# huahbo/IBAMR

Measured on AMD Instinct MI355X. Metric: IB_4 3D spread+interp marker-ops/sec (fp64) + % HBM roofline, 1/2/4/8 GPU, higher is better.
Workload: dtype f64; 1 GPU; cfg4: 1024^3 periodic staggered grid, 1e8 uniform markers (seed 1234), IB_4, z-slabs; kernel=IB_4, markers=100000000, parallelism=z-slab x1, marker_order=cell, layout=packed, spread_mode=one rank, move=False, renumber=False, spread_into=zeroed f (LDataManager::spread, LDataManager.cpp:596), overlap=False

## Files before the change

### ibamr_amd/csrc/le_abi.cpp

```cpp
#include <hip/hip_runtime.h>

#include <algorithm>
#include <climits>
#include <cmath>
#include <cstdlib>
#include <cstdarg>
#include <cstdio>
#include <cstring>
#include <string>
#include <unordered_map>
#include <vector>

#include "../../include/ibtk_le.h"
#include "le_internal.h"

using namespace ibtk_le;

static thread_local std::string g_last_error;

static int fail(int code, const char* fmt, ...) {
    char buf[512];
    va_list ap;
    va_start(ap, fmt);
    vsnprintf(buf, sizeof(buf), fmt, ap);
// ... 129 lines not shown
    int kernel = -1;
    int ndim = 0;
    BinGeom bg{};
    ColGeom cg{};
    int S = 0, nseg = 0;
    ibtk_le_patch_geom geom{};
    DevBuf sorted_key, sorted_l, sorted_s, sorted_X, sorted_a, plane_start, indices, xshift;
    DevBuf sorted_X2, xcur;
    bool xcur_set = false;
    DevBuf lvl_nbr;
    std::vector<int2> lvl_nbr_host;
    DevBuf cand_cnt, cand_off, cand_idx;
    DevBuf last, qdst;
    DevBuf items, nsub, isub, nitems;
    DevBuf cs_cnt, cs_off, cs_pos;
    int cs_state = 0;
    const int* cs_skip = nullptr;
    DevBuf cs_off_z;
    bool cs_split = false;
    long long nclz = 0;
    DevBuf zbits, zst;
    int rb_epoch = 0;
    int item_bound = 0;
    int npatch = 0;
    std::vector<ibtk_le_patch_geom> geoms;
    std::vector<PatchDesc> pdh;
    std::vector<PatchDesc> pdh_dev;
    std::vector<int> off_dev;
    DevBuf pd, entry_off;
    int nbuckets_total = 0, njobs = 0;
// ... 103 lines not shown
extern "C" int ibtk_le_ctx_tune(ibtk_le_ctx ctx, const char* key, int value) {
    if (!ctx || !key) return fail(IBTK_LE_ERR_ARG, "null argument");
    SweepTune& t = ctx->tune;
    const std::string k = key;
    if (k == "seg_items") t.seg_items = value;
    else if (k == "split_target") t.split_target = value;
    else if (k == "heavy") t.heavy = value;
    else if (k == "min_piece") t.min_piece = value;
    else if (k == "heavy_target") t.heavy_target = value;
    else if (k == "heavy_min_piece") t.heavy_min_piece = value;
    else if (k == "heavy_first") t.heavy_first = value;
    else if (k == "strip") t.strip = value;
    else if (k == "xcd_block") t.xcd_block = value;
    else if (k == "interp3") t.interp3 = value;
    else if (k == "side_gather") t.side_gather = value;
    else return fail(IBTK_LE_ERR_ARG, "unknown tuning key %s", key);
    return IBTK_LE_OK;
}

extern "C" int ibtk_le_ctx_enable_timing(ibtk_le_ctx ctx, int enable) {
    if (!ctx) return fail(IBTK_LE_ERR_ARG, "null ctx");
    ctx->timing = enable != 0;
    return IBTK_LE_OK;
}

extern "C" double ibtk_le_ctx_last_kernel_ms(ibtk_le_ctx ctx) {
    if (!ctx || !ctx->ev_valid) return -1.0;
    hipEventSynchronize(ctx->ev1);
    float ms = -1.f;
    if (hipEventElapsedTime(&ms, ctx->ev0, ctx->ev1) != hipSuccess) return -1.0;
// ... 209 lines not shown
    *out = m;
    return IBTK_LE_OK;
}

extern "C" int ibtk_le_markers_destroy(ibtk_le_markers m) {
    if (!m) return IBTK_LE_OK;
    hipSetDevice(m->ctx->device);
    hipStreamSynchronize(m->ctx->stream);
    for (DevBuf* b : {&m->sorted_X2, &m->xcur, &m->lvl_nbr})
        b->release();
    for (DevBuf* b : {&m->sorted_key, &m->sorted_l, &m->sorted_s, &m->sorted_X, &m->sorted_a, &m->plane_start, &m->indices,
                      &m->xshift, &m->cand_cnt, &m->cand_off, &m->cand_idx, &m->last, &m->qdst, &m->items,
                      &m->nsub, &m->isub, &m->nitems, &m->pd, &m->entry_off, &m->qin, &m->owner, &m->int_off,
                      &m->rb_cin, &m->rb_cout, &m->rb_d, &m->rb_dpre, &m->rb_mstart, &m->rb_ps2, &m->rb_mbits,
                      &m->rb_wcnt, &m->rb_wpre, &m->rb_mlist, &m->rb_scr, &m->rb_big, &m->rb_nbig, &m->cs_cnt,
                      &m->cs_off, &m->cs_pos, &m->cs_off_z, &m->zbits, &m->zst, &m->sel_gs})
        b->release();
    delete m;
    return IBTK_LE_OK;
}

extern "C" int ibtk_le_markers_count(ibtk_le_markers m) { return m ? m->n : -1; }

extern "C" int ibtk_le_markers_order(ibtk_le_markers m, const int** order_dev) {
    if (!m || !order_dev) return fail(IBTK_LE_ERR_ARG, "markers_order: null argument");
    *order_dev = m->sorted_l.as<int>();
    return IBTK_LE_OK;
}

#ifndef IBTK_LE_STRIP
#define IBTK_LE_STRIP 1
// ... 525 lines not shown
    if ((rc = m->cand_cnt.ensure(sizeof(int) * (size_t)(items + 1)))) return rc;
    if ((rc = m->cand_off.ensure(sizeof(int) * (size_t)(items + 1)))) return rc;
    if ((rc = m->cand_idx.ensure(sizeof(int) * (size_t)m->n * (m->ndim == 3 ? 8 : 4)))) return rc;
    HIP_TRY(hipMemsetAsync(m->cand_cnt.p, 0, sizeof(int) * (size_t)(items + 1), s));
    HIP_TRY(launch_cand(m->ndim, m->kernel, p, false, m->cand_cnt.as<int>(), nullptr, s));
    size_t tb = 0;
    HIP_TRY(launch_scan(nullptr, tb, m->cand_cnt.as<int>(), m->cand_off.as<int>(), items + 1, s));
    if ((rc = ctx->temp.ensure(tb))) return rc;
    tb = ctx->temp.cap;
    HIP_TRY(launch_scan(ctx->temp.p, tb, m->cand_cnt.as<int>(), m->cand_off.as<int>(), items + 1, s));
    HIP_TRY(launch_cand(m->ndim, m->kernel, p, true, m->cand_off.as<int>(), m->cand_idx.as<int>(), s));
    m->cand_valid = true;
    return IBTK_LE_OK;
}

static bool side_gather(ibtk_le_ctx ctx, ibtk_le_markers m) {
    const int t = ctx->tune.side_gather;
    return t > 0 || (t == 0 && m->n >= (1 << 25));
}
static int gather_fork(ibtk_le_ctx ctx, const Params& p) {
    if (!ctx->side) {
        if (!ctx->ev_fork) HIP_TRY(hipEventCreateWithFlags(&ctx->ev_fork, hipEventDisableTiming));
        if (!ctx->ev_join) HIP_TRY(hipEventCreateWithFlags(&ctx->ev_join, hipEventDisableTiming));
        hipStream_t st = nullptr;
        HIP_TRY(hipStreamCreateWithFlags(&st, hipStreamNonBlocking));
        ctx->side = st;
    }
    HIP_TRY(hipEventRecord(ctx->ev_fork, ctx->stream));
    HIP_TRY(hipStreamWaitEvent(ctx->side, ctx->ev_fork, 0));
    HIP_TRY(launch_gather_F(p, ctx->side));
    HIP_TRY(hipEventRecord(ctx->ev_join, ctx->side));
    return IBTK_LE_OK;
}
// ... 195 lines not shown

extern "C" int ibtk_le_user_interp(ibtk_le_ctx ctx, int centering, int axis, const ibtk_le_patch_geom* geom,
                                   const double* const* q_dev, int q_depth, double* Q_dev, int Q_depth,
                                   const double* X_dev, const int* indices_dev, const double* Xshift_dev, int n) {
    return user_call(ctx, false, centering, axis, geom, const_cast<double* const*>(q_dev), q_depth, Q_dev, Q_depth, X_dev,
                     indices_dev, Xshift_dev, n);
}
extern "C" int ibtk_le_user_spread(ibtk_le_ctx ctx, int centering, int axis, const ibtk_le_patch_geom* geom,
                                   double* const* q_dev, int q_depth, const double* Q_dev, int Q_depth,
                                   const double* X_dev, const int* indices_dev, const double* Xshift_dev, int n) {
    return user_call(ctx, true, centering, axis, geom, q_dev, q_depth, const_cast<double*>(Q_dev), Q_depth, X_dev,
                     indices_dev, Xshift_dev, n);
}

static bool cand_split(int k) { return k == K_IB_4 || k == K_BSPLINE_4 || k == K_IB_6 || k == K_IB_4_W8; }
static bool cand_stream_built(ibtk_le_markers m) {
    return m->cs_state == 1 && m->cs_pos.p && (m->cs_split || !cand_split(m->kernel));
}
static int cand_stream(ibtk_le_ctx ctx, ibtk_le_markers m, Params& p) {
    const long long ncl = (long long)m->nbuckets_total / NBAND;
    const long long nclz = m->npatch ? m->nclz : (long long)m->cg.ncol * (m->cg.nz + 1);
    const int k = m->kernel;
    const bool split = cand_split(k);
    const long long cap = std::min(std::max(4LL * m->n, 1LL), (1LL << 31) - 1);
    if (ncl + 1 >= (1LL << 31) || nclz + 1 >= (1LL << 31))
        return fail(IBTK_LE_ERR_RANGE, "candidate stream too long");
    p.cs_off = m->cs_off.as<int>();
    p.cs_pos = m->cs_pos.as<int>();
    p.cs_total = (int)cap;
    p.cs_off_z = m->cs_split ? m->cs_off_z.as<int>() : nullptr;
    p.cs_rint = k == K_IB_4 ? 1 : 0;
    if (cand_stream_built(m)) return IBTK_LE_OK;
    int rc;
    const size_t tot_at = (sizeof(int) * (size_t)(ncl + 1) + 7) / 8 * 8;
    if ((rc = m->cs_cnt.ensure(tot_at + sizeof(unsigned long long)))) return rc;
    if ((rc = m->cs_off.ensure(sizeof(int) * (size_t)(ncl + 1)))) return rc;
    if ((rc = m->cs_pos.ensure(sizeof(int) * (size_t)cap))) return rc;
    if (split && (rc = m->cs_off_z.ensure(sizeof(int) * (size_t)(nclz + 1)))) return rc;
    p.cs_off = m->cs_off.as<int>();
    p.cs_pos = m->cs_pos.as<int>();
    p.cs_off_z = split ? m->cs_off_z.as<int>() : nullptr;
    HIP_TRY(hipMemsetAsync(m->cs_cnt.as<int>() + ncl, 0, sizeof(int), ctx->stream));
    size_t tb = 0;
    HIP_TRY(launch_scan(nullptr, tb, m->cs_cnt.as<int>(), m->cs_off.as<int>(), (int)(ncl + 1), ctx->stream));
    if ((rc = ctx->temp.ensure(tb))) return rc;
    Params q = p;
    const bool keep = m->cs_state == 2 && (!split || (m->cs_split && m->zst.p));
    q.items_skip = keep ? m->cs_skip : nullptr;
    q.cs_zflip = m->zst.p ? m->zst.as<int>() + 1 : nullptr;
    q.cs_epoch = m->rb_epoch;
    HIP_TRY(launch_cand_stream(q, (int)ncl, m->cs_cnt.as<int>(), m->cs_off.as<int>(), m->cs_pos.as<int>(), ctx->temp.p,
                               ctx->temp.cap,
                               reinterpret_cast<unsigned long long*>(m->cs_cnt.as<char>() + tot_at), ctx->stream));
    m->cs_state = 1;
    m->cs_split = split;
    return IBTK_LE_OK;
}

static int spread_impl(ibtk_le_ctx ctx, ibtk_le_markers m, int kernel, int centering, int axis,
                       const ibtk_le_patch_geom* geom, double* const* q_dev, int q_depth, const double* Q_dev,
                       int Q_depth, const double* ds_dev, const double* X_dev, bool zero_ghosts, bool zero_first) {
    Params p;
    if (int rc = prepare(ctx, m, kernel, geom, X_dev, p)) return rc;
    p.zero_ghosts = zero_ghosts ? 1 : 0;
    p.zero_first = zero_first ? 1 : 0;
    const int nc = ncomponents(geom, centering, q_depth, Q_depth);
    if (nc < 0) return -nc;
    if (m->n == 0) return IBTK_LE_OK;
    if (!Q_dev || !q_dev) return fail(IBTK_LE_ERR_ARG, "null Q or q");
    if (set_device(ctx)) return IBTK_LE_ERR_DEVICE;
    p.Qin = Q_dev;
    p.ds = ds_dev;
    p.Q_depth = Q_depth;
    p.nsorted = m->n;
    {
        if (int rc = ctx->fbuf.ensure(sizeof(double) * (size_t)m->n * (size_t)std::min(nc, MAXC))) return rc;
        p.sorted_F = ctx->fbuf.as<double>();
    }
    if (geom->ndim == 2) {
        if (int rc = build_candidates(ctx, m, p)) return rc;
        p.cand_off = m->cand_off.as<int>();
        p.cand_idx = m->cand_idx.as<int>();
    }
    ctx->ev_valid = false;
    for (int first = 0; first < nc; first += MAXC) {
        const int cnt = std::min(MAXC, nc - first);
        if (int rc = make_comps(geom, centering, axis, q_dev, q_depth, Q_depth, first, cnt, p)) return rc;
        const bool side = geom->ndim == 3 && side_gather(ctx, m) && !cand_stream_built(m);
        if (side)
            if (int rc = gather_fork(ctx, p)) return rc;
        if (geom->ndim == 3)
            if (int rc = cand_stream(ctx, m, p)) return rc;
        if (side)
            if (int rc = gather_join(ctx)) return rc;
        const bool t = ctx->timing && first == 0;
        const size_t nst = (size_t)m->item_bound * cnt * 8;
        if (geom->ndim == 3)
            if (int rc = stamps_begin(ctx, nst, p)) return rc;
        if (geom->ndim == 3) {
            if (int rc = adds_begin(ctx, p, first == 0)) return rc;
            HIP_TRY(launch_spread_sweep(kernel, p, ctx->stream, t ? ctx->ev0 : nullptr, t ? ctx->ev1 : nullptr,
                                        !side));
            if (int rc = adds_end(ctx, p)) return rc;
// ... 294 lines not shown
}

static int level_spread_impl(ibtk_le_ctx ctx, ibtk_le_markers m, int kernel, int centering, int axis,
                             double* const* q_dev, int q_depth, const double* Q_dev, int Q_depth, const double* X_dev,
                             bool zero_first) {
    Params p;
    std::memset(&p, 0, sizeof(p));
    int nc = 0;
    if (int rc = level_params(ctx, m, kernel, centering, axis, q_dev, q_depth, Q_depth, X_dev, false, p, nc))
        return rc;
    if (m->n == 0)
        return zero_first ? ibtk_le_level_zero(ctx, m->npatch, m->geoms.data(), centering, q_dev, q_depth) : IBTK_LE_OK;
    if (!Q_dev) return fail(IBTK_LE_ERR_ARG, "null Q");
    p.Qin = Q_dev;
    p.zero_first = zero_first ? 1 : 0;
    {
        if (int rc = ctx->fbuf.ensure(sizeof(double) * (size_t)m->n * (size_t)nc)) return rc;
        p.sorted_F = ctx->fbuf.as<double>();
    }
    const bool side = side_gather(ctx, m) && !cand_stream_built(m);
    if (side)
        if (int rc = gather_fork(ctx, p)) return rc;
    if (int rc = cand_stream(ctx, m, p)) return rc;
    if (side)
        if (int rc = gather_join(ctx)) return rc;
    const bool t = ctx->timing;
    ctx->ev_valid = false;
    const size_t nst = (size_t)m->item_bound * nc * 8;
    if (int rc = stamps_begin(ctx, nst, p)) return rc;
    if (int rc = adds_begin(ctx, p, true)) return rc;
    HIP_TRY(launch_spread_sweep(kernel, p, ctx->stream, t ? ctx->ev0 : nullptr, t ? ctx->ev1 : nullptr, !side));
    if (int rc = adds_end(ctx, p)) return rc;
    if (int rc = stamps_report(ctx, nst, p)) return rc;
    if (t) ctx->ev_valid = true;
    return IBTK_LE_OK;
// ... 1269 lines not shown
```

### ibamr_amd/csrc/le_internal.h

```cpp
#pragma once
#include <hip/hip_runtime.h>

#include <cstdint>

namespace ibtk_le {

enum : int {
    K_PIECEWISE_CONSTANT = 0,
    K_DISCONTINUOUS_LINEAR = 1,
    K_PIECEWISE_LINEAR = 2,
    K_PIECEWISE_CUBIC = 3,
    K_IB_3 = 4,
    K_IB_4 = 5,
    K_IB_4_W8 = 6,
    K_IB_6 = 7,
    K_BSPLINE_4 = 8,
    K_COUNT = 9
};

struct KernelInfo {
    int W, LO, HI;
};
constexpr KernelInfo kKernelInfo[K_COUNT] = {
    {1, 0, 1},
// ... 53 lines not shown
    int nbuckets;
};

struct SweepTune {
    int seg_items = 0;
    int split_target = 0;
    int heavy = 0;
    int strip = 0;
    int xcd_block = 0;
    int min_piece = 0;
    int heavy_target = 0;
    int heavy_min_piece = 0;
    int heavy_first = 0;
    int interp3 = 0;
    int side_gather = 0;
};
struct SweepItem {
    int col, p0, p1, patch;
};
struct PatchDesc {
    ColGeom cg;
    int bucket_base;
    int ca_base_z;
    int jbase;
    int S, nseg;
    double xlo[3];
    int ilower[3];
    CompDesc comp[MAXC];
};

// ... 21 lines not shown
    double h3;
    double K6;
    const double* X;
    const int* indices;
    const double* Xshift;
    const int* sorted_l;
    const int* sorted_s;
    const double* sorted_X;
    const double* const* sorted_X_ref;
    const unsigned* sorted_key;
    const int* plane_start;
    const int* cand_off;
    const int* cand_idx;
    const int* cs_off;
    const int* cs_pos;
    int cs_total;
    const int* cs_off_z;
    int cs_rint;
    const int* cs_zflip;
    int cs_epoch;
    const int* nentries_dev;
    const double* Qin;
    const double* sorted_F;
    const double* ds;
    int nsorted;
    double* Qout;
    const int* qdst;
    int* err;
    double* sink;
    const int* n_dev = nullptr;
// ... 99 lines not shown
    const void* trec;
    const double *X, *dX, *U;
    double* F;
    int accumulate;
};
hipError_t launch_forcegen(int ndim, const ForceGenParams& p, hipStream_t s);
hipError_t launch_gather_col(int kernel, const Params& p, int n, int* sorted_s, double* sorted_X,
                             const unsigned* sorted_key, int nbuckets, int* bucket_start, hipStream_t s);
hipError_t launch_interp_sweep(int kernel, const Params& p, int n, hipStream_t s, hipEvent_t ev0, hipEvent_t ev1);
hipError_t launch_spread_sweep(int kernel, const Params& p, hipStream_t s, hipEvent_t ev0, hipEvent_t ev1,
                               bool gather = true);
hipError_t launch_gather_F(const Params& p, hipStream_t s);
void sweep_segments(const ColGeom& cg, int& S, int& nseg, int seg_items, bool level);
hipError_t launch_item_table(int kernel, const Params& p, int target, int heavy, int* nsub, int* start, SweepItem* tab, int* ntot,
                             void* temp, size_t temp_bytes, hipStream_t s);
hipError_t launch_cand_stream(const Params& p, int ncl, int* cnt, int* off, int* pos, void* temp, size_t temp_bytes,
                              unsigned long long* total, hipStream_t s);

struct GhostDesc {
    double* u;
    int lo[3], hi[3];
    int ilo[3], ihi[3];
    int64_t s1, s2;
};
constexpr int GSET = 4;
struct GhostSet {
    GhostDesc g[GSET];
};
hipError_t launch_fill_periodic(int ndim, const GhostDesc* g, int n, const int* periodic, hipStream_t s);
hipError_t launch_fold_periodic(int ndim, const GhostDesc* g, int n, const int* periodic, hipStream_t s);
hipError_t launch_zero_ghosts(int ndim, const GhostDesc* g, int n, hipStream_t s);

// ... 133 lines not shown
```

### ibamr_amd/csrc/le_sweep.hip

```cpp
#include <hip/hip_runtime.h>

#include <climits>
#include <type_traits>
#include <cstdio>
#include <cstdlib>

#include "le_internal.h"
#include "le_stencil.h"

namespace ibtk_le {

constexpr int SW = 64;
#ifndef IBTK_LE_DIAG_SPREAD
#define IBTK_LE_DIAG_SPREAD 0
#endif

__device__ __forceinline__ double lds_ld(const double* q) {
    return *(const volatile __attribute__((address_space(3))) double*)q;
}

__device__ __forceinline__ int lane_id() { return __lane_id(); }

struct D3 {
    double v[3];
// ... 1250 lines not shown
            }
        }
        cnt[ca] = t;
    }
}
struct CaJob {
    ColGeom cg;
    int col, a, zb, zilo, o, t;
    double zxlo;
    bool items;
    const int* bs;
    int rowv[3];
    Ranges R;
    int e0;
    double z0;
};
template <bool SHZ>
__global__ __launch_bounds__(BLOCK) void k_cand_write(Params p, int ncl, const int* off, int* pos,
                                                      const unsigned long long* total) {
    if (cs_stands(p)) return;
    if (*total >= (unsigned long long)p.cs_total + 1ull) {
        if (blockIdx.x == 0 && threadIdx.x == 0) atomicOr(p.err, 16);
        return;
    }
    const int lane = threadIdx.x & (SW - 1);
    const int nw = gridDim.x * (BLOCK / SW);
    gdouble* const sX = cur_sorted_X(p);
    const double inv_dz = 1.0 / p.bg.dx[2];
    int* const offz = const_cast<int*>(p.cs_off_z);
    __shared__ int ptab_s[CS_PTAB];
    const int* const ptab = cs_patch_table(p, ptab_s);
    auto load_rows = [&](int ca, CaJob& J) {
        J.items = ca < ncl && ca_decode(p, ca, J.cg, J.col, J.a, J.bs, J.zb, J.zxlo, J.zilo, ptab);
        J.o = off[min(ca, ncl - 1)];
        if (p.pd) J.items = J.items && off[min(ca + 1, ncl)] != J.o;
        if (J.items) {
            const int cx = J.col % J.cg.ncx, cy = J.col / J.cg.ncx;
            const int col0 = (cy - 1) * J.cg.ncx + (cx - 1);
#pragma unroll
            for (int r = 0; r < 3; ++r) J.rowv[r] = J.bs[bucket(J.cg, J.a, col0 + r * J.cg.ncx, 0) + min(lane, 27)];
        }
    };
    auto load_first = [&](CaJob& J) {
        J.t = 0;
        J.e0 = 0;
        J.z0 = 0.0;
        if (!J.items) return;
        make_ranges_lanes(J.rowv, J.R);
        J.t = J.R.pre[SSh<K_IB_4>::NR];
        J.e0 = range_pos(J.R, min(lane, max(J.t - 1, 0)));
        if constexpr (SHZ) J.z0 = sX[(int64_t)3 * min(J.e0, p.nsorted - 1) + 2];
    };
    auto finish = [&](int ca, CaJob& J) {
        if (ca >= ncl) return;
        const int o = J.o;
        if (SHZ && lane == 0) {
            if (J.a == 0) offz[J.zb] = o;
            if (ca == ncl - 1) offz[J.zb + 2] = off[ca + 1];
        }
        const int t = J.t;
        if constexpr (!SHZ) {
            if (lane < t) pos[o + lane] = J.e0;
            for (int j = lane + SW; j < t; j += SW) pos[o + j] = range_pos(J.R, j);
        } else {
            const int aa = J.a + J.cg.org[2] - J.zilo;
            int nlo = 0, nup = 0;
            for (int j0 = 0; j0 < t; j0 += SW) {
                const int j = j0 + lane;
                int e = J.e0;
                double z = J.z0;
                if (j0 > 0) {
                    e = range_pos(J.R, min(j, t - 1));
                    z = sX[(int64_t)3 * e + 2];
                }
                const double xo = (z - J.zxlo) * inv_dz;
                const int n = p.cs_rint ? (int)__builtin_rint(xo) : d_nint(xo);
                const bool in = j < t;
                const bool up = in && n > aa;
                const unsigned long long bu = __ballot(up), bl = __ballot(in && !up);
                const unsigned long long below = (1ull << lane) - 1ull;
                if (in) {
                    if (up) pos[o + t - 1 - (nup + __popcll(bu & below))] = e;
                    else pos[o + nlo + __popcll(bl & below)] = e;
                }
                nlo += __popcll(bl);
                nup += __popcll(bu);
            }
            if (lane == 0) offz[J.zb + 1] = o + nlo;
        }
    };
    for (int ca = blockIdx.x * (BLOCK / SW) + (int)(threadIdx.x / SW); ca < ncl; ca += nw) {
        CaJob J;
        load_rows(ca, J);
        load_first(J);
        finish(ca, J);
    }
}
hipError_t launch_cand_stream(const Params& p, int ncl, int* cnt, int* off, int* pos, void* temp, size_t temp_bytes,
                              unsigned long long* total, hipStream_t s) {
    if (ncl <= 0) return hipSuccess;
    hipLaunchKernelGGL(k_cand_count, dim3(std::min((ncl + BLOCK - 1) / BLOCK, CS_GRID)), dim3(BLOCK), 0, s, p, ncl,
                       cnt);
    hipError_t e = hipMemsetAsync(total, 0, sizeof(unsigned long long), s);
    if (e != hipSuccess) return e;
    if (p.cs_total >= 0x7fffffff && (e = launch_sum64(cnt, ncl, total, s)) != hipSuccess) return e;
    e = launch_scan(temp, temp_bytes, cnt, off, ncl + 1, s);
    if (e != hipSuccess) return e;
    const int per = BLOCK / SW;
    const dim3 g(std::min((ncl + per - 1) / per, CS_GRID)), b(BLOCK);
    if (p.cs_off_z) hipLaunchKernelGGL(k_cand_write<true>, g, b, 0, s, p, ncl, off, pos, total);
    else hipLaunchKernelGGL(k_cand_write<false>, g, b, 0, s, p, ncl, off, pos, total);
    return hipGetLastError();
}

struct Cand {
    double X[3];
    double V;
    int s;
};

template <typename T> __device__ __forceinline__ void rot4(T* w, int r) {
    const bool b0 = r & 1, b1 = r & 2;
    const T c0 = b0 ? w[1] : w[0], c1 = b0 ? w[2] : w[1], c2 = b0 ? w[3] : w[2], c3 = b0 ? w[0] : w[3];
    w[0] = b1 ? c2 : c0;
    w[1] = b1 ? c3 : c1;
    w[2] = b1 ? c0 : c2;
// ... 218 lines not shown
    }
}
template <int K, bool CNT, bool ZC, typename Before>
__device__ __forceinline__ void spread_tiled(const Params& p, const CompDesc& cd, double* ring, const Cand& cdat,
                                             bool act, int a, int X0, int Y0, int zorg, int xlo, int xhi, int ylo,
                                             int yhi, int plo, int phi, double inv_h3, const double* inv_d, Clk& clk,
                                             unsigned long long* cnt, Before&& before) {
    TileAdds<SSh<K, ZC>::W> T;
    spread_setup<K, CNT, ZC>(p, cd, cdat, act, a, X0, Y0, zorg, xlo, xhi, ylo, yhi, plo, phi, inv_h3, inv_d, cnt,
                             before, T);
    clk.lap(2);
    spread_adds<K, ZC>(ring, T);
    clk.lap(3);
}

template <int K, bool LVL, bool CNT, bool ZC>
__global__ __launch_bounds__(SW) void k_spread_sweep(Params p) {
    using S = SSh<K, ZC>;
    constexpr int LO = S::LO, HI = S::HIE, NPL = S::NPL, FAM = S::FAM;
    __shared__ double ring[S::NSL * S::PV];
    const int it = sweep_item(p, p.ncomp);
    if (it < 0) return;
    int c;
    SweepItem si;
    item_decode(p, it, c, si);
    c += p.comp0;
    const int col = si.col;
    const int lane = lane_id();
    ColGeom cg;
    CompDesc cd;
    const int* bs;
// ... 6 lines not shown
    const int zorg = cg.org[2];
    const int xlo = max(cd.lo[0] - X0, 0), xhi = min(cd.hi[0] - X0, COLX - 1);
    const int ylo = max(cd.lo[1] - Y0, 0), yhi = min(cd.hi[1] - Y0, COLY - 1);
    const int plo = max(si.p0, cd.lo[2] - zorg), phi = min(si.p1 - 1, cd.hi[2] - zorg);
    if (xlo > xhi || ylo > yhi || plo > phi) return;
    if (p.zmode) {
        const bool inner = zorg + plo >= p.zlo && zorg + phi <= p.zhi;
        if (inner != (p.zmode == 1)) return;
    }
    const bool shz = FAM == 0 && !cd.zcell;
    static_assert(ZC || FAM != 0, "closed-form kernels: every component on the key-frame ring");
    const int nza = shz ? cg.nz + 1 : cg.nz;
    const int afirst = max(plo - HI, 0), alast = min(phi - LO, nza - 1);
    const int* const cs_offs = shz ? p.cs_off_z : p.cs_off;
    const int ca0 = (LVL ? (shz ? p.pd[si.patch].ca_base_z : p.pd[si.patch].bucket_base / NBAND) : 0) + col * nza + afirst;
    const bool any = cs_offs[ca0 + (alast - afirst + 1)] > cs_offs[ca0];
    const bool zg = p.zero_ghosts && !p.zero_first;
    int dlo[3], dhi[3];
#pragma unroll
    for (int d = 0; d < 3; ++d) {
        dlo[d] = cd.ilower[d];
        dhi[d] = cd.iupper[d];
    }
    const bool xy_inner = X0 >= dlo[0] && X0 + COLX - 1 <= dhi[0] && Y0 >= dlo[1] && Y0 + COLY - 1 <= dhi[1];
    const bool z_inner = zorg + plo >= dlo[2] && zorg + phi <= dhi[2];
    if (!any && !p.zero_first && !(zg && !(xy_inner && z_inner))) return;
    const int nlast = p.nsorted - 1;
    unsigned loff[NPL];
    unsigned gmask = 0;
#pragma unroll
    for (int k = 0; k < NPL; ++k) {
// ... 7 lines not shown
    auto zghost = [&](int z) { return zorg + z < dlo[2] || zorg + z > dhi[2]; };
    const unsigned plane_bytes = (unsigned)(8 * cd.s2);
    auto plane_ptr = [&](int z) {
        const int zc = min(max(zorg + z, cd.lo[2]), cd.hi[2]);
        return plane_rsrc(cd.u + (int64_t)(zc - cd.lo[2]) * cd.s2, plane_bytes);
    };
    if (!any) {
        for (int z = plo; z <= phi; ++z) {
            const auto pb = plane_ptr(z);
            const bool all = p.zero_first || zghost(z);
#pragma unroll
            for (int k = 0; k < NPL; ++k) buf_st(pb, (all || ((gmask >> k) & 1u)) ? loff[k] : OFF_NONE, 0.0);
        }
        return;
    }
    auto cand_at = [&](int e, Cand& d) {
        e = min(max(e, 0), nlast);
#if IBTK_LE_DIAG_SPREAD & 8
        d.X[0] = d.X[1] = d.X[2] = 0.5 + 1e-9 * e;
        d.V = 1.0;
        d.s = 0;
        return;
#endif
        const D3 xs = ld3(sorted_X + (int64_t)3 * e);
        d.X[0] = xs.v[0];
        d.X[1] = xs.v[1];
        d.X[2] = xs.v[2];
        d.V = p.sorted_F[(int64_t)c * p.nsorted + e];
        d.s = FAM == 2 ? p.sorted_s[e] : 0;
    };
    Clk clk;
    unsigned long long cnt[2] = {0ull, 0ull};
    const double inv_h3 = 1.0 / p.h3;
    const double inv_d[3] = {1.0 / p.bg.dx[0], 1.0 / p.bg.dx[1], 1.0 / p.bg.dx[2]};
    auto process = [&](int a, int r, int n, const Cand& mine, auto&& before) {
#if IBTK_LE_DIAG_SPREAD & 4
        asm volatile("" ::"v"(mine.X[0]), "v"(mine.X[1]), "v"(mine.X[2]), "v"(mine.V));
        before();
#else
        spread_tiled<K, CNT, ZC>(p, cd, ring, mine, lane < n, lane < r ? a - 1 : a, X0, Y0, zorg, xlo, xhi, ylo, yhi, plo, phi,
                             inv_h3, inv_d, clk, cnt, before);
#endif
    };
    auto nothing = [] {};
// ... 33 lines not shown
    auto wb_read = [&](int z, double* v) {
        const double* sl = ring + sslot<S>(z) * S::PV;
#pragma unroll
        for (int k = 0; k < NPL; ++k) v[k] = sl[lane + k * SW];
    };
    auto wb_store = [&](int z, bool on, const double* v) {
        const int zc = min(max(zorg + z, cd.lo[2]), cd.hi[2]);
        const bool own = on && z >= plo && z <= phi;
        const auto pb = plane_rsrc(cd.u + (int64_t)(zc - cd.lo[2]) * cd.s2, own ? plane_bytes : 0u);
#pragma unroll
        for (int k = 0; k < NPL; ++k) buf_st(pb, loff[k], v[k]);
    };

    clk.start(p.stamps != nullptr);
    const int* const cs_pos = p.cs_pos;
    const int cs_last = p.cs_total - 1;
    const int nk = alast - afirst + 1;
    auto off_load = [&](int k) { return cs_offs[ca0 + min(k, nk)]; };
    auto pos_load = [&](int j) { return cs_pos[min(max(j, 0), cs_last)]; };
    double pv[NPL] = {};
    for (int z = afirst + LO; z < afirst + HI; ++z) {
        plane_load(z, pv);
        plane_put(z, pv);
    }
    plane_load(afirst + HI, pv);
    int O0 = __builtin_amdgcn_readfirstlane(off_load(0)), O1 = __builtin_amdgcn_readfirstlane(off_load(1));
    int O2 = __builtin_amdgcn_readfirstlane(off_load(2)), O3 = __builtin_amdgcn_readfirstlane(off_load(3));
    int O4v = off_load(4);
    int R0 = 0;
    int N0 = min(O1 - O0, SW);
    int R1 = (O1 - O0 - N0) % SW;
    int N1 = R1 + min(SW - R1, O2 - O1);
    Cand nxt, nxt2;
    {
        const int e0 = pos_load(O0 + min(lane, max(N0 - 1, 0)));
        cand_at(e0, nxt);
    }
    int I1 = pos_load(O1 - R1 + min(lane, max(N1 - 1, 0)));
    clk.lap(0);
    auto anchor_step = [&](int a, const Cand& cur, Cand& nxt) __attribute__((always_inline)) {
        const int k = a - afirst;
        const int zw = a - 2 + LO;
        double wb[NPL];
        wb_read(zw, wb);
        plane_put(a + HI, pv);
        asm volatile("" ::"v"(cur.X[0]), "v"(cur.X[1]), "v"(cur.X[2]), "v"(cur.V), "v"(I1), "v"(O4v));
        const int O4 = __builtin_amdgcn_readfirstlane(O4v);
        const int cur_r = R0, cur_n = N0;
        const int tCur = O1 - O0;
        const int h = min(SW - R0, tCur);
        const int nmid = (tCur - h) / SW;
        const int r_a = R1;
        clk.lap(1);
        int R2 = 0, N2 = 0;
        if (a + 1 <= alast) {
            cand_at(I1, nxt);
            const int t1 = O2 - O1;
            R2 = (t1 - min(SW - R1, t1)) % SW;
            N2 = R2 + min(SW - R2, O3 - O2);
            I1 = pos_load(O2 - R2 + min(lane, max(N2 - 1, 0)));
            O4v = off_load(k + 5);
            plane_load(a + HI + 1, pv);
        }
        const bool wbon = a >= afirst + 2;
        if (cur_n > 0) process(a, cur_r, cur_n, cur, [&] { wb_store(zw, wbon, wb); });
        else wb_store(zw, wbon, wb);
        if (nmid > 0) {
            const int mbase = O0 + h + lane;
            Cand more, more2;
            cand_at(pos_load(mbase), more);
            int m = 0;
            if constexpr (PAIR) {
                if (nmid > 1) cand_at(pos_load(mbase + SW), more2);
                int q2 = pos_load(mbase + SW * 2), q3 = pos_load(mbase + SW * 3);
                for (; m + 1 < nmid; m += 2) {
                    const Cand n0 = more, n1 = more2;
                    if (m + 2 < nmid) cand_at(q2, more);
                    if (m + 3 < nmid) cand_at(q3, more2);
                    q2 = pos_load(mbase + SW * (m + 4));
                    q3 = pos_load(mbase + SW * (m + 5));
                    process2(a, n0, n1);
                }
            }
            int q1 = pos_load(mbase + SW * (m + 1));
            for (; m < nmid; ++m) {
                const Cand now = more;
                if (m + 1 < nmid) cand_at(q1, more);
                q1 = pos_load(mbase + SW * (m + 2));
                process(a, 0, SW, now, nothing);
            }
        }
        if (a == alast && r_a > 0) {
            Cand last;
            cand_at(pos_load(O1 - r_a + min(lane, r_a - 1)), last);
            process(a, 0, r_a, last, nothing);
        }
        R0 = R1;
        N0 = N1;
        R1 = R2;
        N1 = N2;
        O0 = O1;
        O1 = O2;
        O2 = O3;
        O3 = O4;
        clk.lap(4);
    };
    for (int a = afirst; a <= alast; ++a) {
        anchor_step(a, nxt, nxt2);
        nxt = nxt2;
// ... 248 lines not shown
    }
}

hipError_t launch_gather_F(const Params& p, hipStream_t s) {
    if (p.nsorted > 0) {
        const bool rec3 = p.ncomp == 3 && p.Q_depth == 3 && p.comp[0].qcomp == 0 && p.comp[1].qcomp == 1 &&
                          p.comp[2].qcomp == 2;
        const dim3 g((p.nsorted + BLOCK - 1) / BLOCK), b(BLOCK);
        if (rec3) hipLaunchKernelGGL(k_gather_F_col<true>, g, b, 0, s, p, p.nsorted, const_cast<double*>(p.sorted_F));
        else hipLaunchKernelGGL(k_gather_F_col<false>, g, b, 0, s, p, p.nsorted, const_cast<double*>(p.sorted_F));
    }
    return hipGetLastError();
}
template <int K>
hipError_t launch_spread_sweep_t(const Params& p, hipStream_t s, hipEvent_t ev0, hipEvent_t ev1, bool gather) {
    if (gather)
        if (hipError_t e = launch_gather_F(p, s); e != hipSuccess) return e;
    if (ev0) (void)hipEventRecord(ev0, s);
    const long items = (long)p.item_bound * p.ncomp;
    if (items > 0) {
        Params q = p;
        q.comp0 = 0;
        const dim3 g(sweep_grid(q, items)), b(SW);
        constexpr bool ZC = KT<K>::FAM == 0;
        if (q.nadd) {
            if (q.pd) hipLaunchKernelGGL((k_spread_sweep<K, true, true, ZC>), g, b, 0, s, q);
            else hipLaunchKernelGGL((k_spread_sweep<K, false, true, ZC>), g, b, 0, s, q);
        } else {
            if (q.pd) hipLaunchKernelGGL((k_spread_sweep<K, true, false, ZC>), g, b, 0, s, q);
            else hipLaunchKernelGGL((k_spread_sweep<K, false, false, ZC>), g, b, 0, s, q);
        }
    }
    if (ev1) (void)hipEventRecord(ev1, s);
    return hipGetLastError();
}

#define IBTK_LE_DISPATCH_K(KV, CALL)                                 \
    switch (KV) {                                                    \
    case K_PIECEWISE_CONSTANT: return CALL<K_PIECEWISE_CONSTANT>;    \
    case K_DISCONTINUOUS_LINEAR: return CALL<K_DISCONTINUOUS_LINEAR>; \
    case K_PIECEWISE_LINEAR: return CALL<K_PIECEWISE_LINEAR>;        \
    case K_PIECEWISE_CUBIC: return CALL<K_PIECEWISE_CUBIC>;          \
    case K_IB_3: return CALL<K_IB_3>;                                \
    case K_IB_4: return CALL<K_IB_4>;                                \
    case K_IB_4_W8: return CALL<K_IB_4_W8>;                          \
    case K_IB_6: return CALL<K_IB_6>;                                \
// ... 100 lines not shown
```

Measured before the change: 8.330 billion marker-ops/s.

## Stream marker source indices in candidate list to skip separate force gather pass

The candidate-stream builder now also records each candidate's original marker index (cs_src). The spread sweep kernel, under a new FS template flag, reads force values straight from Qin (scaled by ds) through that index, so the separate gather pass into sorted_F and its side-stream overlap are dropped. It is on by default (f_stream defaults to 0, so the test >= 0 holds). This saves one pass that writes and then rereads an n×ncomp buffer. In exchange it adds an extra int stream load per candidate and turns coalesced sorted reads into scattered reads of Qin.

```diff
diff --git a/ibamr_amd/csrc/le_abi.cpp b/ibamr_amd/csrc/le_abi.cpp
--- a/ibamr_amd/csrc/le_abi.cpp
+++ b/ibamr_amd/csrc/le_abi.cpp
@@ -167,6 +167,8 @@
     DevBuf last, qdst;
     DevBuf items, nsub, isub, nitems;
     DevBuf cs_cnt, cs_off, cs_pos;
+    DevBuf cs_src;
+    bool cs_has_src = false;
     int cs_state = 0;
     const int* cs_skip = nullptr;
     DevBuf cs_off_z;
@@ -300,6 +302,7 @@
     else if (k == "xcd_block") t.xcd_block = value;
     else if (k == "interp3") t.interp3 = value;
     else if (k == "side_gather") t.side_gather = value;
+    else if (k == "f_stream") t.f_stream = value;
     else return fail(IBTK_LE_ERR_ARG, "unknown tuning key %s", key);
     return IBTK_LE_OK;
 }
@@ -539,7 +542,7 @@
                       &m->nsub, &m->isub, &m->nitems, &m->pd, &m->entry_off, &m->qin, &m->owner, &m->int_off,
                       &m->rb_cin, &m->rb_cout, &m->rb_d, &m->rb_dpre, &m->rb_mstart, &m->rb_ps2, &m->rb_mbits,
                       &m->rb_wcnt, &m->rb_wpre, &m->rb_mlist, &m->rb_scr, &m->rb_big, &m->rb_nbig, &m->cs_cnt,
-                      &m->cs_off, &m->cs_pos, &m->cs_off_z, &m->zbits, &m->zst, &m->sel_gs})
+                      &m->cs_off, &m->cs_pos, &m->cs_src, &m->cs_off_z, &m->zbits, &m->zst, &m->sel_gs})
         b->release();
     delete m;
     return IBTK_LE_OK;
@@ -1095,9 +1098,12 @@
     return IBTK_LE_OK;
 }
 
+static bool f_stream(ibtk_le_ctx ctx, ibtk_le_markers) {
+    return ctx->tune.f_stream >= 0;
+}
 static bool side_gather(ibtk_le_ctx ctx, ibtk_le_markers m) {
     const int t = ctx->tune.side_gather;
-    return t > 0 || (t == 0 && m->n >= (1 << 25));
+    return !f_stream(ctx, m) && (t > 0 || (t == 0 && m->n >= (1 << 25)));
 }
 static int gather_fork(ibtk_le_ctx ctx, const Params& p) {
     if (!ctx->side) {
@@ -1323,46 +1329,51 @@
 }
 
 static bool cand_split(int k) { return k == K_IB_4 || k == K_BSPLINE_4 || k == K_IB_6 || k == K_IB_4_W8; }
-static bool cand_stream_built(ibtk_le_markers m) {
-    return m->cs_state == 1 && m->cs_pos.p && (m->cs_split || !cand_split(m->kernel));
+static bool cand_stream_built(ibtk_le_markers m, bool src) {
+    return m->cs_state == 1 && m->cs_pos.p && (m->cs_split || !cand_split(m->kernel)) && (!src || m->cs_has_src);
 }
 static int cand_stream(ibtk_le_ctx ctx, ibtk_le_markers m, Params& p) {
     const long long ncl = (long long)m->nbuckets_total / NBAND;
     const long long nclz = m->npatch ? m->nclz : (long long)m->cg.ncol * (m->cg.nz + 1);
     const int k = m->kernel;
     const bool split = cand_split(k);
+    const bool src = f_stream(ctx, m);
     const long long cap = std::min(std::max(4LL * m->n, 1LL), (1LL << 31) - 1);
     if (ncl + 1 >= (1LL << 31) || nclz + 1 >= (1LL << 31))
         return fail(IBTK_LE_ERR_RANGE, "candidate stream too long");
     p.cs_off = m->cs_off.as<int>();
     p.cs_pos = m->cs_pos.as<int>();
+    p.cs_src = src ? m->cs_src.as<int>() : nullptr;
     p.cs_total = (int)cap;
     p.cs_off_z = m->cs_split ? m->cs_off_z.as<int>() : nullptr;
     p.cs_rint = k == K_IB_4 ? 1 : 0;
-    if (cand_stream_built(m)) return IBTK_LE_OK;
+    if (cand_stream_built(m, src)) return IBTK_LE_OK;
     int rc;
     const size_t tot_at = (sizeof(int) * (size_t)(ncl + 1) + 7) / 8 * 8;
     if ((rc = m->cs_cnt.ensure(tot_at + sizeof(unsigned long long)))) return rc;
     if ((rc = m->cs_off.ensure(sizeof(int) * (size_t)(ncl + 1)))) return rc;
     if ((rc = m->cs_pos.ensure(sizeof(int) * (size_t)cap))) return rc;
+    if (src && (rc = m->cs_src.ensure(sizeof(int) * (size_t)cap))) return rc;
     if (split && (rc = m->cs_off_z.ensure(sizeof(int) * (size_t)(nclz + 1)))) return rc;
     p.cs_off = m->cs_off.as<int>();
     p.cs_pos = m->cs_pos.as<int>();
+    p.cs_src = src ? m->cs_src.as<int>() : nullptr;
     p.cs_off_z = split ? m->cs_off_z.as<int>() : nullptr;
     HIP_TRY(hipMemsetAsync(m->cs_cnt.as<int>() + ncl, 0, sizeof(int), ctx->stream));
     size_t tb = 0;
     HIP_TRY(launch_scan(nullptr, tb, m->cs_cnt.as<int>(), m->cs_off.as<int>(), (int)(ncl + 1), ctx->stream));
     if ((rc = ctx->temp.ensure(tb))) return rc;
     Params q = p;
-    const bool keep = m->cs_state == 2 && (!split || (m->cs_split && m->zst.p));
+    const bool keep = m->cs_state == 2 && (!split || (m->cs_split && m->zst.p)) && (!src || m->cs_has_src);
     q.items_skip = keep ? m->cs_skip : nullptr;
     q.cs_zflip = m->zst.p ? m->zst.as<int>() + 1 : nullptr;
     q.cs_epoch = m->rb_epoch;
-    HIP_TRY(launch_cand_stream(q, (int)ncl, m->cs_cnt.as<int>(), m->cs_off.as<int>(), m->cs_pos.as<int>(), ctx->temp.p,
-                               ctx->temp.cap,
+    HIP_TRY(launch_cand_stream(q, (int)ncl, m->cs_cnt.as<int>(), m->cs_off.as<int>(), m->cs_pos.as<int>(),
+                               src ? m->cs_src.as<int>() : nullptr, ctx->temp.p, ctx->temp.cap,
                                reinterpret_cast<unsigned long long*>(m->cs_cnt.as<char>() + tot_at), ctx->stream));
     m->cs_state = 1;
     m->cs_split = split;
+    m->cs_has_src = src;
     return IBTK_LE_OK;
 }
 
@@ -1382,7 +1393,8 @@
     p.ds = ds_dev;
     p.Q_depth = Q_depth;
     p.nsorted = m->n;
-    {
+    p.sorted_F = nullptr;
+    if (geom->ndim == 2 || !f_stream(ctx, m)) {
         if (int rc = ctx->fbuf.ensure(sizeof(double) * (size_t)m->n * (size_t)std::min(nc, MAXC))) return rc;
         p.sorted_F = ctx->fbuf.as<double>();
     }
@@ -1395,7 +1407,7 @@
     for (int first = 0; first < nc; first += MAXC) {
         const int cnt = std::min(MAXC, nc - first);
         if (int rc = make_comps(geom, centering, axis, q_dev, q_depth, Q_depth, first, cnt, p)) return rc;
-        const bool side = geom->ndim == 3 && side_gather(ctx, m) && !cand_stream_built(m);
+        const bool side = geom->ndim == 3 && side_gather(ctx, m) && !cand_stream_built(m, false);
         if (side)
             if (int rc = gather_fork(ctx, p)) return rc;
         if (geom->ndim == 3)
@@ -1720,11 +1732,12 @@
     if (!Q_dev) return fail(IBTK_LE_ERR_ARG, "null Q");
     p.Qin = Q_dev;
     p.zero_first = zero_first ? 1 : 0;
-    {
+    p.sorted_F = nullptr;
+    if (!f_stream(ctx, m)) {
         if (int rc = ctx->fbuf.ensure(sizeof(double) * (size_t)m->n * (size_t)nc)) return rc;
         p.sorted_F = ctx->fbuf.as<double>();
     }
-    const bool side = side_gather(ctx, m) && !cand_stream_built(m);
+    const bool side = side_gather(ctx, m) && !cand_stream_built(m, false);
     if (side)
         if (int rc = gather_fork(ctx, p)) return rc;
     if (int rc = cand_stream(ctx, m, p)) return rc;
diff --git a/ibamr_amd/csrc/le_internal.h b/ibamr_amd/csrc/le_internal.h
--- a/ibamr_amd/csrc/le_internal.h
+++ b/ibamr_amd/csrc/le_internal.h
@@ -91,6 +91,7 @@
     int heavy_first = 0;
     int interp3 = 0;
     int side_gather = 0;
+    int f_stream = 0;
 };
 struct SweepItem {
     int col, p0, p1, patch;
@@ -142,6 +143,7 @@
     const int* cand_idx;
     const int* cs_off;
     const int* cs_pos;
+    const int* cs_src = nullptr;
     int cs_total;
     const int* cs_off_z;
     int cs_rint;
@@ -271,8 +273,8 @@
 void sweep_segments(const ColGeom& cg, int& S, int& nseg, int seg_items, bool level);
 hipError_t launch_item_table(int kernel, const Params& p, int target, int heavy, int* nsub, int* start, SweepItem* tab, int* ntot,
                              void* temp, size_t temp_bytes, hipStream_t s);
-hipError_t launch_cand_stream(const Params& p, int ncl, int* cnt, int* off, int* pos, void* temp, size_t temp_bytes,
-                              unsigned long long* total, hipStream_t s);
+hipError_t launch_cand_stream(const Params& p, int ncl, int* cnt, int* off, int* pos, int* src, void* temp,
+                              size_t temp_bytes, unsigned long long* total, hipStream_t s);
 
 struct GhostDesc {
     double* u;
diff --git a/ibamr_amd/csrc/le_sweep.hip b/ibamr_amd/csrc/le_sweep.hip
--- a/ibamr_amd/csrc/le_sweep.hip
+++ b/ibamr_amd/csrc/le_sweep.hip
@@ -1288,13 +1288,17 @@
     Ranges R;
     int e0;
     double z0;
+    int s0;
 };
 template <bool SHZ>
-__global__ __launch_bounds__(BLOCK) void k_cand_write(Params p, int ncl, const int* off, int* pos,
+__global__ __launch_bounds__(BLOCK) void k_cand_write(Params p, int ncl, const int* off, int* pos, int* src,
                                                       const unsigned long long* total) {
     if (cs_stands(p)) return;
     if (*total >= (unsigned long long)p.cs_total + 1ull) {
         if (blockIdx.x == 0 && threadIdx.x == 0) atomicOr(p.err, 16);
+        if (src)
+            for (int64_t j = (int64_t)blockIdx.x * BLOCK + threadIdx.x; j < p.cs_total; j += (int64_t)gridDim.x * BLOCK)
+                src[j] = 0;
         return;
     }
     const int lane = threadIdx.x & (SW - 1);
@@ -1319,11 +1323,13 @@
         J.t = 0;
         J.e0 = 0;
         J.z0 = 0.0;
+        J.s0 = 0;
         if (!J.items) return;
         make_ranges_lanes(J.rowv, J.R);
         J.t = J.R.pre[SSh<K_IB_4>::NR];
         J.e0 = range_pos(J.R, min(lane, max(J.t - 1, 0)));
         if constexpr (SHZ) J.z0 = sX[(int64_t)3 * min(J.e0, p.nsorted - 1) + 2];
+        if (src) J.s0 = p.sorted_s[min(J.e0, p.nsorted - 1)];
     };
     auto finish = [&](int ca, CaJob& J) {
         if (ca >= ncl) return;
@@ -1336,16 +1342,21 @@
         if constexpr (!SHZ) {
             if (lane < t) pos[o + lane] = J.e0;
             for (int j = lane + SW; j < t; j += SW) pos[o + j] = range_pos(J.R, j);
+            if (src) {
+                if (lane < t) src[o + lane] = J.s0;
+                for (int j = lane + SW; j < t; j += SW) src[o + j] = p.sorted_s[min(range_pos(J.R, j), p.nsorted - 1)];
+            }
         } else {
             const int aa = J.a + J.cg.org[2] - J.zilo;
             int nlo = 0, nup = 0;
             for (int j0 = 0; j0 < t; j0 += SW) {
                 const int j = j0 + lane;
-                int e = J.e0;
+                int e = J.e0, ms = J.s0;
                 double z = J.z0;
                 if (j0 > 0) {
                     e = range_pos(J.R, min(j, t - 1));
                     z = sX[(int64_t)3 * e + 2];
+                    if (src) ms = p.sorted_s[min(e, p.nsorted - 1)];
                 }
                 const double xo = (z - J.zxlo) * inv_dz;
                 const int n = p.cs_rint ? (int)__builtin_rint(xo) : d_nint(xo);
@@ -1354,8 +1365,9 @@
                 const unsigned long long bu = __ballot(up), bl = __ballot(in && !up);
                 const unsigned long long below = (1ull << lane) - 1ull;
                 if (in) {
-                    if (up) pos[o + t - 1 - (nup + __popcll(bu & below))] = e;
-                    else pos[o + nlo + __popcll(bl & below)] = e;
+                    const int at = up ? o + t - 1 - (nup + __popcll(bu & below)) : o + nlo + __popcll(bl & below);
+                    pos[at] = e;
+                    if (src) src[at] = ms;
                 }
                 nlo += __popcll(bl);
                 nup += __popcll(bu);
@@ -1370,8 +1382,8 @@
         finish(ca, J);
     }
 }
-hipError_t launch_cand_stream(const Params& p, int ncl, int* cnt, int* off, int* pos, void* temp, size_t temp_bytes,
-                              unsigned long long* total, hipStream_t s) {
+hipError_t launch_cand_stream(const Params& p, int ncl, int* cnt, int* off, int* pos, int* src, void* temp,
+                              size_t temp_bytes, unsigned long long* total, hipStream_t s) {
     if (ncl <= 0) return hipSuccess;
     hipLaunchKernelGGL(k_cand_count, dim3(std::min((ncl + BLOCK - 1) / BLOCK, CS_GRID)), dim3(BLOCK), 0, s, p, ncl,
                        cnt);
@@ -1382,8 +1394,8 @@
     if (e != hipSuccess) return e;
     const int per = BLOCK / SW;
     const dim3 g(std::min((ncl + per - 1) / per, CS_GRID)), b(BLOCK);
-    if (p.cs_off_z) hipLaunchKernelGGL(k_cand_write<true>, g, b, 0, s, p, ncl, off, pos, total);
-    else hipLaunchKernelGGL(k_cand_write<false>, g, b, 0, s, p, ncl, off, pos, total);
+    if (p.cs_off_z) hipLaunchKernelGGL(k_cand_write<true>, g, b, 0, s, p, ncl, off, pos, src, total);
+    else hipLaunchKernelGGL(k_cand_write<false>, g, b, 0, s, p, ncl, off, pos, src, total);
     return hipGetLastError();
 }
 
@@ -1632,7 +1644,7 @@
     clk.lap(3);
 }
 
-template <int K, bool LVL, bool CNT, bool ZC>
+template <int K, bool LVL, bool CNT, bool ZC, bool FS>
 __global__ __launch_bounds__(SW) void k_spread_sweep(Params p) {
     using S = SSh<K, ZC>;
     constexpr int LO = S::LO, HI = S::HIE, NPL = S::NPL, FAM = S::FAM;
@@ -1669,7 +1681,8 @@
     const int afirst = max(plo - HI, 0), alast = min(phi - LO, nza - 1);
     const int* const cs_offs = shz ? p.cs_off_z : p.cs_off;
     const int ca0 = (LVL ? (shz ? p.pd[si.patch].ca_base_z : p.pd[si.patch].bucket_base / NBAND) : 0) + col * nza + afirst;
-    const bool any = cs_offs[ca0 + (alast - afirst + 1)] > cs_offs[ca0];
+    const int o_end = cs_offs[ca0 + (alast - afirst + 1)];
+    const bool any = o_end > cs_offs[ca0];
     const bool zg = p.zero_ghosts && !p.zero_first;
     int dlo[3], dhi[3];
 #pragma unroll
@@ -1707,7 +1720,8 @@
         }
         return;
     }
-    auto cand_at = [&](int e, Cand& d) {
+    const int* const cs_src = p.cs_src;
+    auto cand_at = [&](int e, int s, Cand& d) {
         e = min(max(e, 0), nlast);
 #if IBTK_LE_DIAG_SPREAD & 8
         d.X[0] = d.X[1] = d.X[2] = 0.5 + 1e-9 * e;
@@ -1719,8 +1733,14 @@
         d.X[0] = xs.v[0];
         d.X[1] = xs.v[1];
         d.X[2] = xs.v[2];
-        d.V = p.sorted_F[(int64_t)c * p.nsorted + e];
-        d.s = FAM == 2 ? p.sorted_s[e] : 0;
+        if constexpr (FS) {
+            const double v = p.Qin[(int64_t)p.Q_depth * s + cd.qcomp];
+            d.V = p.ds ? v * p.ds[s] : v;
+            d.s = FAM == 2 ? s : 0;
+        } else {
+            d.V = p.sorted_F[(int64_t)c * p.nsorted + e];
+            d.s = FAM == 2 ? p.sorted_s[e] : 0;
+        }
     };
     Clk clk;
     unsigned long long cnt[2] = {0ull, 0ull};
@@ -1784,10 +1804,14 @@
 
     clk.start(p.stamps != nullptr);
     const int* const cs_pos = p.cs_pos;
-    const int cs_last = p.cs_total - 1;
     const int nk = alast - afirst + 1;
     auto off_load = [&](int k) { return cs_offs[ca0 + min(k, nk)]; };
+    const int cs_last = max(min(p.cs_total, __builtin_amdgcn_readfirstlane(o_end)) - 1, 0);
     auto pos_load = [&](int j) { return cs_pos[min(max(j, 0), cs_last)]; };
+    auto src_load = [&](int j) {
+        if constexpr (FS) return cs_src[min(max(j, 0), cs_last)];
+        else return 0;
+    };
     double pv[NPL] = {};
     for (int z = afirst + LO; z < afirst + HI; ++z) {
         plane_load(z, pv);
@@ -1803,10 +1827,12 @@
     int N1 = R1 + min(SW - R1, O2 - O1);
     Cand nxt, nxt2;
     {
-        const int e0 = pos_load(O0 + min(lane, max(N0 - 1, 0)));
-        cand_at(e0, nxt);
+        const int j0 = O0 + min(lane, max(N0 - 1, 0));
+        const int e0 = pos_load(j0);
+        cand_at(e0, src_load(j0), nxt);
     }
     int I1 = pos_load(O1 - R1 + min(lane, max(N1 - 1, 0)));
+    int S1 = src_load(O1 - R1 + min(lane, max(N1 - 1, 0)));
     clk.lap(0);
     auto anchor_step = [&](int a, const Cand& cur, Cand& nxt) __attribute__((always_inline)) {
         const int k = a - afirst;
@@ -1815,6 +1841,7 @@
         wb_read(zw, wb);
         plane_put(a + HI, pv);
         asm volatile("" ::"v"(cur.X[0]), "v"(cur.X[1]), "v"(cur.X[2]), "v"(cur.V), "v"(I1), "v"(O4v));
+        if constexpr (FS) asm volatile("" ::"v"(S1));
         const int O4 = __builtin_amdgcn_readfirstlane(O4v);
         const int cur_r = R0, cur_n = N0;
         const int tCur = O1 - O0;
@@ -1824,11 +1851,12 @@
         clk.lap(1);
         int R2 = 0, N2 = 0;
         if (a + 1 <= alast) {
-            cand_at(I1, nxt);
+            cand_at(I1, S1, nxt);
             const int t1 = O2 - O1;
             R2 = (t1 - min(SW - R1, t1)) % SW;
             N2 = R2 + min(SW - R2, O3 - O2);
             I1 = pos_load(O2 - R2 + min(lane, max(N2 - 1, 0)));
+            S1 = src_load(O2 - R2 + min(lane, max(N2 - 1, 0)));
             O4v = off_load(k + 5);
             plane_load(a + HI + 1, pv);
         }
@@ -1838,31 +1866,35 @@
         if (nmid > 0) {
             const int mbase = O0 + h + lane;
             Cand more, more2;
-            cand_at(pos_load(mbase), more);
+            cand_at(pos_load(mbase), src_load(mbase), more);
             int m = 0;
             if constexpr (PAIR) {
-                if (nmid > 1) cand_at(pos_load(mbase + SW), more2);
+                if (nmid > 1) cand_at(pos_load(mbase + SW), src_load(mbase + SW), more2);
                 int q2 = pos_load(mbase + SW * 2), q3 = pos_load(mbase + SW * 3);
+                int s2 = src_load(mbase + SW * 2), s3 = src_load(mbase + SW * 3);
                 for (; m + 1 < nmid; m += 2) {
                     const Cand n0 = more, n1 = more2;
-                    if (m + 2 < nmid) cand_at(q2, more);
-                    if (m + 3 < nmid) cand_at(q3, more2);
+                    if (m + 2 < nmid) cand_at(q2, s2, more);
+                    if (m + 3 < nmid) cand_at(q3, s3, more2);
                     q2 = pos_load(mbase + SW * (m + 4));
                     q3 = pos_load(mbase + SW * (m + 5));
+                    s2 = src_load(mbase + SW * (m + 4));
+                    s3 = src_load(mbase + SW * (m + 5));
                     process2(a, n0, n1);
                 }
             }
-            int q1 = pos_load(mbase + SW * (m + 1));
+            int q1 = pos_load(mbase + SW * (m + 1)), s1 = src_load(mbase + SW * (m + 1));
             for (; m < nmid; ++m) {
                 const Cand now = more;
-                if (m + 1 < nmid) cand_at(q1, more);
+                if (m + 1 < nmid) cand_at(q1, s1, more);
                 q1 = pos_load(mbase + SW * (m + 2));
+                s1 = src_load(mbase + SW * (m + 2));
                 process(a, 0, SW, now, nothing);
             }
         }
         if (a == alast && r_a > 0) {
             Cand last;
-            cand_at(pos_load(O1 - r_a + min(lane, r_a - 1)), last);
+            cand_at(pos_load(O1 - r_a + min(lane, r_a - 1)), src_load(O1 - r_a + min(lane, r_a - 1)), last);
             process(a, 0, r_a, last, nothing);
         }
         R0 = R1;
@@ -2141,7 +2173,7 @@
 }
 template <int K>
 hipError_t launch_spread_sweep_t(const Params& p, hipStream_t s, hipEvent_t ev0, hipEvent_t ev1, bool gather) {
-    if (gather)
+    if (gather && !p.cs_src)
         if (hipError_t e = launch_gather_F(p, s); e != hipSuccess) return e;
     if (ev0) (void)hipEventRecord(ev0, s);
     const long items = (long)p.item_bound * p.ncomp;
@@ -2150,13 +2182,18 @@
         q.comp0 = 0;
         const dim3 g(sweep_grid(q, items)), b(SW);
         constexpr bool ZC = KT<K>::FAM == 0;
-        if (q.nadd) {
-            if (q.pd) hipLaunchKernelGGL((k_spread_sweep<K, true, true, ZC>), g, b, 0, s, q);
-            else hipLaunchKernelGGL((k_spread_sweep<K, false, true, ZC>), g, b, 0, s, q);
-        } else {
-            if (q.pd) hipLaunchKernelGGL((k_spread_sweep<K, true, false, ZC>), g, b, 0, s, q);
-            else hipLaunchKernelGGL((k_spread_sweep<K, false, false, ZC>), g, b, 0, s, q);
-        }
+        auto launch = [&](auto fs) {
+            constexpr bool FS = decltype(fs)::value;
+            if (q.nadd) {
+                if (q.pd) hipLaunchKernelGGL((k_spread_sweep<K, true, true, ZC, FS>), g, b, 0, s, q);
+                else hipLaunchKernelGGL((k_spread_sweep<K, false, true, ZC, FS>), g, b, 0, s, q);
+            } else {
+                if (q.pd) hipLaunchKernelGGL((k_spread_sweep<K, true, false, ZC, FS>), g, b, 0, s, q);
+                else hipLaunchKernelGGL((k_spread_sweep<K, false, false, ZC, FS>), g, b, 0, s, q);
+            }
+        };
+        if (q.cs_src) launch(std::true_type{});
+        else launch(std::false_type{});
     }
     if (ev1) (void)hipEventRecord(ev1, s);
     return hipGetLastError();
```

Measured after the change: 8.530 billion marker-ops/s, median of 6. 1.02x the previous value.
